# audeering/opensmile

Hardware: NVIDIA H100
Metric: LLD frames/sec (16kHz, 25ms/10ms) (higher is better)
Workload: dtype f32

## Files before the change

### opensmile_b200/csrc/api.cu

```cuda
#include <cuda_runtime.h>

#include <algorithm>
#include <cmath>
#include <cstdio>
#include <cstdlib>
#include <cstring>
#include <memory>
#include <string>
#include <vector>

#include "cuda_owned.hpp"
#include "kernels.cuh"
#include "plan.hpp"

using namespace osm;

namespace osm {
cudaError_t launch_lld_f32(const LldParams &p, int nfft, int numSMs, cudaStream_t st, LldLaunchInfo *info);
cudaError_t launch_energy_f32(const TimeOpParams &p, cudaStream_t st);
cudaError_t launch_mzcr_f32(const TimeOpParams &p, cudaStream_t st);
cudaError_t launch_intensity_f32(const TimeOpParams &p, cudaStream_t st);
cudaError_t launch_formant_f32(const FormantParams &p, cudaStream_t st);
cudaError_t launch_lpc_f32(const LpcParams &p, cudaStream_t st);
size_t lpc_smem_bytes_f32(const LpcParams &p);
cudaError_t launch_jitter_f32(const JitterParams &p, int u0, int u1, cudaStream_t st);
}

namespace {
thread_local std::string g_err;
}
namespace osm { osm_b200_status set_last_error(osm_b200_status st, const std::string &msg) { g_err = msg; return st; } }

namespace {
// ... 67 lines not shown
  RastaParams rp;
  DevBuf<float> dBand;
};

struct StreamRt {
  LldParams kp;
  std::vector<PassRt> extra;
  PassRt pass0x;
  int tileF = 32;
  bool runLld = false;
  bool forceNarrow = false;
  bool needTiles = false;
  const float *dWindow = nullptr;
  std::vector<int32_t> uttChunk0, uttTile0;
  PinBuf<ChunkRef> hChunks; DevBuf<ChunkRef> dChunks; size_t nChunks = 0;
  PinBuf<OpTile> hTiles; DevBuf<OpTile> dTiles; size_t nTiles = 0;
  DevBuf<float> dMag;
};

struct OpRt {
  int kind = 0, stream = 0;
  int vSrcCol = 0, vN = 0, vOutCol = 0;
  int magMode = 0; float magN = 1.f, magDbNorm = 0.f, magMinDb = 0.f;
  SpectralParams sp;
  TimeOpParams tp;
  AcfPitchParams ap;
  DevBuf<double> dSharpW;
  DevBuf<float2> dTw;
  DevBuf<PitchRaw> dRaw;
  ShsParams shs;
// ... 814 lines not shown
      size_t ti = 0;
      if (needPost)
        for (int u = 0; u < nUtt; u++) {
          const int64_t To = hR[u + 1] - hR[u];
          for (int64_t r0 = 0; r0 < To; r0 += PR) pl->hPost.p[ti++] = TileRef{u, (int32_t)r0};
        }
    }
    pl->nPostTiles = nPost;
    pl->totalWork = 0;
    for (size_t si = 0; si < pl->st.size(); si++) {
      StreamRt &rt = pl->st[si];
      const int F = rt.tileF, H = rt.kp.halo;
      std::vector<ChunkRef> chunks;
      std::vector<OpTile> tiles;
      rt.uttChunk0.assign(nm, 0); rt.uttTile0.assign(nm, 0);
      int64_t tileCount = 0;
      for (int u = 0; u < nUtt; u++) {
        const int64_t L = uttOff[u + 1] - uttOff[u];
        const int64_t T = desc_num_static_frames(d, (int)si, L);
        rt.uttChunk0[u] = (int32_t)chunks.size();
        rt.uttTile0[u] = (int32_t)tileCount;
        for (int64_t a = 0; a < T;) {
          const int64_t s0 = std::max<int64_t>(a - H, 0);
          const int64_t maxEnd = s0 + (int64_t)F * KT;
          const int64_t b2 = (maxEnd >= T) ? T : maxEnd - H;
          chunks.push_back(ChunkRef{u, (int32_t)a, (int32_t)b2, (int32_t)(tileCount + s0 / F)});
          a = b2;
        }
        if (rt.needTiles)
          for (int64_t f0 = 0; f0 < T; f0 += F)
            tiles.push_back(OpTile{u, (int32_t)f0, (int32_t)std::min<int64_t>(F, T - f0), f0 > 0 ? 1 : 0});
        tileCount += (T + F - 1) / F;
      }
      rt.uttChunk0[nUtt] = (int32_t)chunks.size();
      rt.uttTile0[nUtt] = (int32_t)tileCount;
      rt.nChunks = rt.runLld ? chunks.size() : 0;
      rt.nTiles = tiles.size();
      pl->totalWork += rt.nChunks + rt.nTiles;
      if (rt.runLld) {
        CU(rt.hChunks.reserve(chunks.size() + 1));
        if (!chunks.empty()) memcpy(rt.hChunks.p, chunks.data(), chunks.size() * sizeof(ChunkRef));
        CU(rt.dChunks.reserve(chunks.size() + 1));
        if (!chunks.empty()) CU(cudaMemcpyAsync(rt.dChunks.p, rt.hChunks.p, chunks.size() * sizeof(ChunkRef), cudaMemcpyHostToDevice, st));
        if (rt.kp.opKind < 0 || d.streams[si].dumpMag)
          CU(rt.dMag.reserve((size_t)tileCount * d.streams[si].fe.nBins * F + 64));
      }
      if (rt.needTiles) {
        CU(rt.hTiles.reserve(tiles.size() + 1));
        if (!tiles.empty()) memcpy(rt.hTiles.p, tiles.data(), tiles.size() * sizeof(OpTile));
        CU(rt.dTiles.reserve(tiles.size() + 1));
        if (!tiles.empty()) CU(cudaMemcpyAsync(rt.dTiles.p, rt.hTiles.p, tiles.size() * sizeof(OpTile), cudaMemcpyHostToDevice, st));
      }
    }
    pl->totalRows = hR[nUtt];
    pl->totalStat = hS[nUtt];
    pl->totalSamples = uttOff[nUtt];
    CU(pl->dMeta.reserve(3 * nm));
    CU(pl->dPost.reserve(nPost + 1));
    CU(cudaMemcpyAsync(pl->dMeta.p, pl->hMeta.p, 3 * nm * sizeof(long long), cudaMemcpyHostToDevice, st));
    if (nPost) CU(cudaMemcpyAsync(pl->dPost.p, pl->hPost.p, nPost * sizeof(TileRef), cudaMemcpyHostToDevice, st));
// ... 48 lines not shown
  }
  for (size_t si = 0; si < pl->st.size(); si++) {
    StreamRt &rt = pl->st[si];
    if (!rt.runLld) continue;
    const int c0 = rt.uttChunk0[u0], c1 = rt.uttChunk0[u1];
    if (c1 <= c0) continue;
    const long long *hS = pl->hMeta.p + 2 * nm;
    const long long row0 = hS[u0], row1 = hS[u1];
    for (size_t j = 0; j <= rt.extra.size(); j++) {
      PassRt &pr = j == 0 ? rt.pass0x : rt.extra[j - 1];
      LldParams kp = j == 0 ? rt.kp : pr.kp;
      kp.pcm = reinterpret_cast<const int16_t *>(d_pcm);
      kp.uttOff = dU;
      kp.chunks = rt.dChunks.p + c0;
      kp.nChunks = c1 - c0;
      kp.magOut = (j == 0 && d.streams[si].dumpMag) ? rt.dMag.p : nullptr;
      if (pl->staticDirect) {
        kp.out = d_out; kp.outStride = d.nOut; kp.outCol = pl->identityOutCol; kp.rowOff = dR;
      } else {
        kp.out = pl->dStat.p; kp.outStride = d.nStatic; kp.rowOff = dS;
        kp.outCol = pr.op >= 0 ? d.ops[pr.op].outCol : 0;
      }
      if (pr.rasta) {
        CU(pr.dBand.reserve((size_t)pl->totalStat * kp.nBands + 64));
        kp.out = pr.dBand.p; kp.outStride = kp.nBands; kp.outCol = 0; kp.rowOff = dS;
      }
      CU((f32in ? launch_lld_f32 : launch_lld)(kp, d.streams[si].fe.nfft, pl->numSMs, st, &pl->lastInfo));
      pl->lastLaunches++;
      PROF("lld_kernel");
      if (pr.rasta) {
        RastaParams rp = pr.rp;
        rp.band = pr.dBand.p; rp.uttOff = dU; rp.statOff = dS;
        CU(launch_rasta(rp, u0, u1, st));
        PROF("rasta_kernel");
        CU(launch_plp_tail(pr.tail, pr.dBand.p, pl->dStat.p, d.nStatic, d.ops[pr.op].outCol, row0, row1, st));
        pl->lastLaunches += 2;
        PROF("plp_tail_kernel");
      }
    }
  }
  if (u0 == 0) CU(cudaEventRecord(pl->evKm, st));
  bool forked = false;
// ... 334 lines not shown
```

### opensmile_b200/csrc/kernels.cu

```cuda
#include <cstdio>
#include <cstdlib>
#include <string>

#include "fft_radix.cuh"
#include "kernels.cuh"

#include "lld_common.cuh"

namespace osm {

constexpr int kUnrollMel = OSM_UNROLL_MEL, kUnrollDct = OSM_UNROLL_DCT;

template <int M, int F, int NT, int MINB, bool VEC2, bool GEN>
__global__ void __launch_bounds__(NT, MINB) lld_kernel(const LldParams p)
{
  const int opKind = GEN ? p.opKind : 0;
  float *const magOut = GEN ? p.magOut : nullptr;
  constexpr int NW = NT / 32, G = 32 / F, NVW = NW * G;
  constexpr int NBINS = M + 1;
  constexpr int NPAIR = M / 2 + 1;
  constexpr int PAIRS_PER_VW = (NPAIR + NVW - 1) / NVW;
  using Fc = Fact<M>;

  extern __shared__ __align__(16) unsigned char smem[];
// ... 9 lines not shown
  float2 *sSplit = reinterpret_cast<float2 *>(smem + L.splitTw);
  float2 *sMelCoef = reinterpret_cast<float2 *>(smem + L.melCoef);
  int *sMelRange = reinterpret_cast<int *>(smem + L.melRange);
  float *sDct = reinterpret_cast<float *>(smem + L.dctCos);
  float *sLift = reinterpret_cast<float *>(smem + L.dctLift);
  float *sEql = reinterpret_cast<float *>(smem + L.eql);
  float *melS = reinterpret_cast<float *>(smem + L.melS);
  float *ring = reinterpret_cast<float *>(smem + L.ring);
  float *Dbuf = reinterpret_cast<float *>(smem + L.zbuf);

  const int tid = threadIdx.x;
  const int warp = tid >> 5, lane = tid & 31;
  const int f = lane & (F - 1);
  const int vw = warp * G + lane / F;

  if (tid == 0) mbar_init(mbar, 1);
  for (int i = tid; i < M; i += NT) sWinLut[i] = p.winLut[i];
  for (int i = tid; i < p.twCount; i += NT) sTw[i] = p.twiddles[i];
  for (int i = tid; i < NPAIR; i += NT) sSplit[i] = p.splitTw[i];
  if (opKind >= 0) {
    for (int i = tid; i < p.melVCount; i += NT) sMelCoef[i] = p.melVisit[i];
    for (int i = tid; i < p.nBands + 2; i += NT) { sMelRange[i] = p.melRange[i]; sMelRange[p.nBands + 2 + i] = p.melVB[i]; }
    for (int i = tid; i < p.dctRows * p.dctStride; i += NT) sDct[i] = p.dctCos[i];
    if (opKind == 1) for (int i = tid; i < p.nBands; i += NT) sEql[i] = p.plpEql[i];
    for (int i = tid; i < p.nStat; i += NT) sLift[i] = p.dctLift[i];
  }
  for (int i = tid; i < L.sampFloats; i += NT) samp[i] = 0.f;
  for (int i = tid; i < F; i += NT) raw[i] = 0.f;
  __syncthreads();

  const int hop = p.frameStep, nChan = p.nChan;
  const int S = hop + p.sPad;
  uint32_t phase = 0;

  int chunk = blockIdx.x;
  if (chunk >= p.nChunks) return;
  ChunkCtx cx = load_chunk<F>(p, chunk);
  int j = 0;
  int emitted = cx.a;
  if (tid == 0) {
    const TileGeom g0 = tile_geom<F>(p, cx, 0);
    mbar_expect_tx(mbar, g0.bytes);
    bulk_g2s(rawPcm, g0.src, g0.bytes, mbar);
  }

  while (chunk < p.nChunks) {
    const TileGeom tg = tile_geom<F>(p, cx, j);
    const int nf = tg.nf, count = tg.count;

    mbar_wait(mbar, phase);
    phase ^= 1;
    {
      const int16_t *rp = reinterpret_cast<const int16_t *>(rawPcm + tg.mis) + tg.lead * nChan;
      const bool fastLoad = (tg.mis == 0) && (nChan <= 2) && !(OSM_PCM_F32_SUPPORT && p.pcmF32);
      const bool fastStore = (p.sPad == 0) || (hop % 8 == 0);
      for (int c = tid; c * 8 < count; c += NT) {
        const int i = c * 8;
        const int nvalid = min(8, count - i);
        float x[8];
        if (fastLoad && nvalid == 8) {
          if (nChan == 1) {
// ... 47 lines not shown
              if (rr == 0 && qq < F) raw[qq] = x[jj];
              dst[jj] = y[jj];
              rr++;
              if (rr == hop) { rr = 0; qq++; dst += p.sPad; }
            }
          }
        }
      }
    }
    __syncthreads();
    if (tid == 0) {
      if (j + 1 < cx.nT) {
        const TileGeom gn = tile_geom<F>(p, cx, j + 1);
        mbar_expect_tx(mbar, gn.bytes);
        bulk_g2s(rawPcm, gn.src, gn.bytes, mbar);
      } else if (chunk + (int)gridDim.x < p.nChunks) {
        const ChunkCtx cn = load_chunk<F>(p, chunk + gridDim.x);
        const TileGeom gn = tile_geom<F>(p, cn, 0);
        mbar_expect_tx(mbar, gn.bytes);
        bulk_g2s(rawPcm, gn.src, gn.bytes, mbar);
      }
    }

    {
      const float *sampF = samp + f * S;
      fft_stage<M, F, NVW, Fc::R0, M, true, false, VEC2>(Z, sampF, raw, sWinLut, sTw + p.twOff[0], p, vw, f);
      __syncthreads();
      if constexpr (Fc::NS == 2) {
        fft_stage<M, F, NVW, Fc::R1, M / Fc::R0, false, true, VEC2>(Z, nullptr, nullptr, nullptr, nullptr, p, vw, f);
      } else {
        fft_stage<M, F, NVW, Fc::R1, M / Fc::R0, false, false, VEC2>(Z, nullptr, nullptr, nullptr, sTw + p.twOff[1], p, vw, f);
        __syncthreads();
// ... 169 lines not shown
      } else {
        emit_edge<F, NW>(ring, Dbuf, outS, K, W1, W2, T, T1, c01, c02, cx.s0, r0, r1, d0, d1, dRows, norm1, p.fRcp1, norm2, p.fRcp2, warp, lane);
      }
      {
        float *o = p.out + (cx.row0 + r0) * (long long)K3;
        const int n = nr * K3;
        for (int i = tid; i < n; i += NT) o[i] = outS[i];
      }
      emitted = r1;
    }

    }

    j++;
    if (j == cx.nT) {
      chunk += gridDim.x;
      j = 0;
      if (chunk < p.nChunks) { cx = load_chunk<F>(p, chunk); emitted = cx.a; }
    }
  }
}

constexpr int kPostRows = 64;
constexpr int kPostMaxHalo = 12;
constexpr int kPostThreads = 256;

__device__ __forceinline__ float post_read(const float *lvl, int n, int rowBase, int t, int W, int navail, int i, int c)
{
  if (t - W < 0) {
    if (i < 0) i = 0;
    else if (i >= navail) return 0.f;
  } else if (i > navail - 1) {
    i = navail - 1;
// ... 357 lines not shown
  return (size_t)make_layout(p, nfft / 2, lld_tile_frames(nfft, p.narrow != 0)).total;
}

#define OSM_STR2(x) #x
#define OSM_STR(x) OSM_STR2(x)
template <int M, int F, int NT, int MINB, bool VEC2, bool GEN>
static const char *lld_kernel_name()
{
  static const std::string name = std::string(OSM_STR(lld_kernel)) + "<" + std::to_string(M) + "," + std::to_string(F) + "," +
                                  std::to_string(NT) + "," + std::to_string(MINB) + (VEC2 ? ",VEC2" : ",SCALAR") +
                                  (GEN ? ",GEN>" : ",MFCC>");
  return name.c_str();
}

template <int M, int F, int NT, int MINB, bool VEC2, bool GEN>
static cudaError_t launch_g(const LldParams &p, int numSMs, cudaStream_t st, LldLaunchInfo *info)
{
  const size_t smem = (size_t)make_layout(p, M, F).total;
  auto kern = lld_kernel<M, F, NT, MINB, VEC2, GEN>;
  cudaError_t e = cudaFuncSetAttribute(kern, cudaFuncAttributeMaxDynamicSharedMemorySize, (int)smem);
  if (e != cudaSuccess) return e;
  int occ = 0;
  e = cudaOccupancyMaxActiveBlocksPerMultiprocessor(&occ, kern, NT, smem);
  if (e != cudaSuccess) return e;
  if (occ < 1) return cudaErrorLaunchOutOfResources;
  int grid = numSMs * occ;
  if (grid > p.nChunks) grid = p.nChunks;
  if (grid < 1) grid = 1;
  if (info) {
    info->grid = grid; info->block = NT; info->smem = smem; info->nChunks = p.nChunks;
    info->kernel = lld_kernel_name<M, F, NT, MINB, VEC2, GEN>();
  }
  kern<<<grid, NT, smem, st>>>(p);
  return cudaGetLastError();
}

template <int M, int F, int NT, int MINB, bool VEC2>
static cudaError_t launch_t(const LldParams &p, int numSMs, cudaStream_t st, LldLaunchInfo *info)
{
  if (p.opKind == 0 && p.magOut == nullptr) return launch_g<M, F, NT, MINB, VEC2, false>(p, numSMs, st, info);
  return launch_g<M, F, NT, MINB, VEC2, true>(p, numSMs, st, info);
}

cudaError_t launch_lld(const LldParams &p, int nfft, int numSMs, cudaStream_t st, LldLaunchInfo *info)
{
  {
    static const bool fastOn = [] { const char *e = getenv("OSM_B200_LLD_FAST"); return !(e && e[0] == '0'); }();
    if (fastOn && lld_fast_applies(p, nfft)) return launch_lld_fast(p, numSMs, st, info);
  }
  const bool vec2 = ((p.frameStep + p.sPad) % 2) == 0;
  if (p.narrow && nfft == 1024) return vec2 ? launch_t<512, 16, 256, 1, true>(p, numSMs, st, info) : launch_t<512, 16, 256, 1, false>(p, numSMs, st, info);
  if (p.narrow && nfft == 2048) return vec2 ? launch_t<1024, 8, 256, 1, true>(p, numSMs, st, info) : launch_t<1024, 8, 256, 1, false>(p, numSMs, st, info);
  if (p.narrow && nfft == 4096) return vec2 ? launch_t<2048, 4, 128, 1, true>(p, numSMs, st, info) : launch_t<2048, 4, 128, 1, false>(p, numSMs, st, info);
  switch (nfft) {
    case 512:  return vec2 ? launch_t<256, 32, 256, 2, true>(p, numSMs, st, info) : launch_t<256, 32, 256, 2, false>(p, numSMs, st, info);
    case 1024: return vec2 ? launch_t<512, 32, 512, 1, true>(p, numSMs, st, info) : launch_t<512, 32, 512, 1, false>(p, numSMs, st, info);
    case 2048: return vec2 ? launch_t<1024, 16, 512, 1, true>(p, numSMs, st, info) : launch_t<1024, 16, 512, 1, false>(p, numSMs, st, info);
    case 4096: return vec2 ? launch_t<2048, 8, 256, 1, true>(p, numSMs, st, info) : launch_t<2048, 8, 256, 1, false>(p, numSMs, st, info);
    default:   return cudaErrorInvalidValue;
  }
}

int post_tile_rows(int nStat, int maxN, int halo)
{
  int rows = kPostRows;
  while (rows > 4 && (size_t)(rows + 2 * halo) * (nStat + 2 * maxN) * sizeof(float) > 160 * 1024) rows /= 2;
  return rows;
}

cudaError_t launch_post(const PostParams &p, cudaStream_t st)
{
  if (p.nTiles <= 0 || p.nGroups <= 0) return cudaSuccess;
  if (p.halo > kPostMaxHalo) return cudaErrorInvalidValue;
// ... 191 lines not shown
```

### opensmile_b200/csrc/kernels.cuh

```cuda
#pragma once
#include <cuda_runtime.h>
#include <cstdint>

#ifdef OSM_F32_VARIANT
#define OSM_PCM_F32_SUPPORT 1
#define lld_tile_frames lld_tile_frames_f32
#define lld_virtual_warps lld_virtual_warps_f32
#define lld_max_chunk_tiles lld_max_chunk_tiles_f32
#define lld_supported_fft lld_supported_fft_f32
#define lld_smem_bytes lld_smem_bytes_f32
#define launch_lld launch_lld_f32
#define post_tile_rows post_tile_rows_f32
#define launch_post launch_post_f32
#define acf_pitch_supported_fft acf_pitch_supported_fft_f32
#define launch_acf_pitch launch_acf_pitch_f32
#define launch_rasta launch_rasta_f32
#define launch_plp_tail launch_plp_tail_f32
#define launch_cms_means launch_cms_means_f32
#define launch_vecop_ll1 launch_vecop_ll1_f32
#define launch_pitch_smooth launch_pitch_smooth_f32
#define launch_spectral launch_spectral_f32
#define launch_mag_rows launch_mag_rows_f32
#define launch_intensity launch_intensity_f32
#define launch_energy launch_energy_f32
// ... 17 lines not shown
#define plp_tail_kernel plp_tail_kernel_f32
#define post_kernel post_kernel_f32
#define rasta_kernel rasta_kernel_f32
#define spectral_kernel spectral_kernel_f32
#define vecop_ll1_kernel vecop_ll1_kernel_f32
#endif
#ifndef OSM_PCM_F32_SUPPORT
#define OSM_PCM_F32_SUPPORT 0
#endif

namespace osm {

constexpr int kMaxVW = 32;

struct TileRef { int32_t utt; int32_t f0; };
struct ChunkRef { int32_t utt; int32_t a; int32_t b; int32_t tile0; };

struct LldParams {
  const int16_t *pcm;
  const long long *uttOff;
  const long long *rowOff;
  const ChunkRef *chunks;
  int nChunks;
  int nChan;
  int pcmF32;
  unsigned hopMagic;
  int narrow;
  int fused, halo, fW1, fW2;
  float fNorm1, fNorm2;
  float fRcp1, fRcp2;
  int frameSize, frameStep, sPad;
  int preemph, preDe;
  float preK, oneMinusK;
  int hasWinOffset;
  float winOffset;
  const float4 *winLut;
  const float2 *twiddles;
  int twOff[4];
// ... 42 lines not shown
  const long long *uttOff;
  int nUtt;
  int nGroups;
  PostGroup groups[kMaxPostGroups];
  const TileRef *tiles;
  int rows;
  int nTiles;
  int nStat;
  int maxN;
  int halo;
  const float *means;
};

struct LldLaunchInfo { int grid, block; size_t smem; const char *kernel; long long nChunks; };

cudaError_t launch_lld(const LldParams &p, int nfft, int numSMs, cudaStream_t st, LldLaunchInfo *info);
cudaError_t launch_post(const PostParams &p, cudaStream_t st);
bool lld_fast_applies(const LldParams &p, int nfft);
cudaError_t launch_lld_fast(const LldParams &p, int numSMs, cudaStream_t st, LldLaunchInfo *info);
int post_tile_rows(int nStat, int maxN, int halo);
size_t lld_smem_bytes(const LldParams &p, int nfft);
int lld_tile_frames(int nfft, bool narrow = false);
int lld_virtual_warps(int nfft);
int lld_max_chunk_tiles();
bool lld_supported_fft(int nfft);

struct OpTile { int32_t utt; int32_t f0; int32_t nf; int32_t prev; };

struct SpectralParams {
  const float *mag;
  const OpTile *tiles; int nTiles; int F;
  const long long *statOff;
  float *stat; int statStride, outCol;
  int nSrc, loBin, hiBin;
// ... 165 lines not shown
```

### opensmile_b200/csrc/lld_common.cuh

```cuda
#pragma once
#include <cstdio>

#include "fft_radix.cuh"
#include "kernels.cuh"

#ifndef OSM_EMIT_LANES
#define OSM_EMIT_LANES 0
#endif
#ifndef OSM_MEL_COMPACT
#define OSM_MEL_COMPACT 1
#endif
#ifndef OSM_UNROLL_MEL
#define OSM_UNROLL_MEL 4
#endif
#ifndef OSM_UNROLL_DCT
#define OSM_UNROLL_DCT 2
#endif

namespace osm {

struct SmemLayout {
  int zbuf, samp, raw, rawPcm, mbar, winLut, tw, splitTw, melCoef, melRange, dctCos, dctLift, eql, melS, ring;
  int total;
  int sampFloats, rawPcmBytes;
// ... 98 lines not shown
__device__ __forceinline__ ChunkCtx load_chunk(const LldParams &p, int chunk)
{
  ChunkCtx c;
  const ChunkRef cr = p.chunks[chunk];
  c.utt = cr.utt; c.a = cr.a; c.b = cr.b; c.tile0 = cr.tile0;
  c.uo = p.uttOff[cr.utt];
  const long long Ls = p.uttOff[cr.utt + 1] - c.uo;
  c.T = (int)((Ls - p.frameSize) / p.frameStep + 1);
  c.s0 = max(cr.a - p.halo, 0);
  c.sEnd = min(cr.b + p.halo, c.T);
  c.nT = (c.sEnd - c.s0 + F - 1) / F;
  c.row0 = p.rowOff[cr.utt];
  return c;
}

struct TileGeom {
  int fs;
  int nf;
  int count;
  int lead;
  int mis;
  uint32_t bytes;
  const char *src;
};

template <int F>
__device__ __forceinline__ TileGeom tile_geom(const LldParams &p, const ChunkCtx &c, int j)
{
  TileGeom g;
  g.fs = c.s0 + j * F;
// ... 286 lines not shown
```

### opensmile_b200/csrc/lld_fast.cu

```cuda
#include "lld_common.cuh"

#ifndef OSM_FAST_FUSED_DCT
#define OSM_FAST_FUSED_DCT 0
#endif
#ifndef OSM_FAST_P1_UNROLL
#define OSM_FAST_P1_UNROLL 1
#endif
#ifndef OSM_FAST_P2_UNROLL
#define OSM_FAST_P2_UNROLL 2
#endif
#ifndef OSM_FAST_MEL_UNROLL
#define OSM_FAST_MEL_UNROLL 1
#endif
#ifndef OSM_FAST_DCT_UNROLL
#define OSM_FAST_DCT_UNROLL 4
#endif
#ifndef OSM_FAST_STAGE_UNROLL
#define OSM_FAST_STAGE_UNROLL 1
#endif
#ifndef OSM_FAST_EMIT_K13
#define OSM_FAST_EMIT_K13 0
#endif
#define OSM_PRAGMA_(x) _Pragma(#x)
#define OSM_UNROLL(n) OSM_PRAGMA_(unroll n)

namespace osm {
namespace {

constexpr int kM = 256, kF = 32, kNT = 256, kNW = 8;
constexpr int kKMax = 16;
constexpr int kPartOff = 9216;

__device__ __forceinline__ void dft4_d0(float2 &a, float2 &b, float2 &c, float2 &d)
{
  const float2 t0 = cadd(a, c), t1 = csub(a, c), bb = b;
  a = cadd(t0, bb);
  c = csub(t0, bb);
  b = make_float2(t1.x + bb.y, t1.y - bb.x);
  d = make_float2(t1.x - bb.y, t1.y + bb.x);
}

// ... 32 lines not shown
  const float2 t2 = cmul(o2, w);
  const float xr = e2.x + t2.y, xi = e2.y - t2.x;
  const float yr = e2.x - t2.y, yi = e2.y + t2.x;
  pk = __fmaf_rn(xr, xr, __fmul_rn(xi, xi));
  pm = __fmaf_rn(yr, yr, __fmul_rn(yi, yi));
}

template <int NZR>
__global__ void __launch_bounds__(kNT, 2) lld512_kernel(const LldParams p)
{
  constexpr int M = kM, F = kF, NT = kNT, NW = kNW;
  using D16 = Dft<16>;

  extern __shared__ __align__(16) unsigned char smem[];
  __shared__ ChunkCtx sCx[2];
  const SmemLayout L = make_layout(p, M, F);
  float2 *Z = reinterpret_cast<float2 *>(smem + L.zbuf);
  float *P = reinterpret_cast<float *>(smem + L.zbuf);
  float *samp = reinterpret_cast<float *>(smem + L.samp);
  float *raw = reinterpret_cast<float *>(smem + L.raw);
  unsigned char *rawPcm = smem + L.rawPcm;
  uint64_t *mbar = reinterpret_cast<uint64_t *>(smem + L.mbar);
  float4 *sWinLut = reinterpret_cast<float4 *>(smem + L.winLut);
  float2 *sTw = reinterpret_cast<float2 *>(smem + L.tw);
  float2 *sSplit = reinterpret_cast<float2 *>(smem + L.splitTw);
  float2 *sMelCoef = reinterpret_cast<float2 *>(smem + L.melCoef);
  int *sMelRange = reinterpret_cast<int *>(smem + L.melRange);
  float *sDct = reinterpret_cast<float *>(smem + L.dctCos);
  float *sLift = reinterpret_cast<float *>(smem + L.dctLift);
  float *ring = reinterpret_cast<float *>(smem + L.ring);
  float *Dbuf = reinterpret_cast<float *>(smem + L.zbuf);

  const int tid = threadIdx.x;
  const int warp = tid >> 5, f = tid & 31;

  if (tid == 0) mbar_init(mbar, 1);
  for (int i = tid; i < M; i += NT) sWinLut[i] = p.winLut[i];
  for (int i = tid; i < p.twCount; i += NT) sTw[i] = p.twiddles[i];
  for (int i = tid; i < M / 2 + 1; i += NT) sSplit[i] = p.splitTw[i];
  for (int i = tid; i < p.melVCount; i += NT) sMelCoef[i] = p.melVisit[i];
  for (int i = tid; i < p.nBands + 2; i += NT) { sMelRange[i] = p.melRange[i]; sMelRange[p.nBands + 2 + i] = p.melVB[i]; }
  for (int i = tid; i < p.nBands * kKMax; i += NT) {
    const int m = i / kKMax, c = i - m * kKMax;
    sDct[i] = (c < p.nStat) ? p.dctCos[c * p.dctStride + m] : 0.f;
  }
  for (int i = tid; i < p.nStat; i += NT) sLift[i] = p.dctLift[i];
  for (int i = tid; i < L.sampFloats; i += NT) samp[i] = 0.f;
  for (int i = tid; i < F; i += NT) raw[i] = 0.f;
  __syncthreads();

  const int hop = p.frameStep;
  const int S = hop + p.sPad;
  uint32_t phase = 0;

  int chunk = blockIdx.x;
  if (chunk >= p.nChunks) return;
  int cpar = 0;
  if (tid == 0) {
    sCx[0] = load_chunk<F>(p, chunk);
    const TileGeom g0 = tile_geom<F>(p, sCx[0], 0);
    mbar_expect_tx(mbar, g0.bytes);
    bulk_g2s(rawPcm, g0.src, g0.bytes, mbar);
  }
  __syncthreads();
  int j = 0;
  int emitted = sCx[0].a;

  const int tA = (warp == 0) ? 0 : warp, tB = (warp == 0) ? 8 : 16 - warp;
  const int wl = (warp == 0) ? 8 : warp, wh = (warp == 0) ? 0 : warp;
  const int melBs = p.melSplit[warp], melBe = p.melSplit[warp + 1];

  while (chunk < p.nChunks) {
    const ChunkCtx &cx = sCx[cpar];

    mbar_wait(mbar, phase);
    phase ^= 1;
    {
      const TileGeom tg = tile_geom<F>(p, cx, j);
      const int count = tg.count;
      const int16_t *rp = reinterpret_cast<const int16_t *>(rawPcm + tg.mis) + tg.lead;
      const bool aligned = (tg.mis == 0);
      const bool hasLead = tg.lead > 0;
      const float ks = p.preDe ? p.preK : -p.preK;
      OSM_UNROLL(OSM_FAST_STAGE_UNROLL)
      for (int i = tid * 8; i < count; i += NT * 8) {
        int wds[4];
        if (aligned) {
// ... 20 lines not shown
          for (int jj = 0; jj < 8; jj++) y[jj] = x[jj];
        }
        const int q = (int)__umulhi((unsigned)i, p.hopMagic);
        float *dst = samp + i + q * p.sPad;
        if (i == q * hop && q < F) raw[q] = x[0];
#pragma unroll
        for (int jj = 0; jj < 8; jj += 2) *reinterpret_cast<float2 *>(dst + jj) = make_float2(y[jj], y[jj + 1]);
      }
    }
    __syncthreads();
    if (tid == 0) {
      if (j + 1 < cx.nT) {
        const TileGeom gn = tile_geom<F>(p, cx, j + 1);
        mbar_expect_tx(mbar, gn.bytes);
        bulk_g2s(rawPcm, gn.src, gn.bytes, mbar);
      } else if (chunk + (int)gridDim.x < p.nChunks) {
        const ChunkCtx cn = load_chunk<F>(p, chunk + gridDim.x);
        sCx[cpar ^ 1] = cn;
        const TileGeom gn = tile_geom<F>(p, cn, 0);
        mbar_expect_tx(mbar, gn.bytes);
        bulk_g2s(rawPcm, gn.src, gn.bytes, mbar);
      }
    }

    {
      const float *sampF = samp + f * S;
      const float2 *tw0 = sTw + p.twOff[0];
      OSM_UNROLL(OSM_FAST_P1_UNROLL)
      for (int t = warp; t < 16; t += NW) {
        float2 v[16];
#pragma unroll
        for (int r = 0; r < 16; r++) {
          if (r < NZR) {
            const float4 wl = sWinLut[t + 16 * r];
            const float2 x = *reinterpret_cast<const float2 *>(sampF + __float_as_int(wl.z));
            v[r] = make_float2(__fmul_rn(x.x, wl.x), __fmul_rn(x.y, wl.y));
          } else {
            v[r] = make_float2(0.f, 0.f);
          }
        }
        if (t == 0 && p.preemph)
          v[0].x = __fmul_rn(__fmul_rn(p.oneMinusK, raw[f]), sWinLut[0].x);
        dft16_first<NZR>(v);
        const float2 *twj = tw0 + t * 16;
#pragma unroll
        for (int q = 1; q < 16; q++) v[D16::out(q)] = cmul(v[D16::out(q)], twj[q]);
        float2 *zp = Z + t * F + f;
#pragma unroll
        for (int q = 0; q < 16; q++) zp[(16 * q) * F] = v[D16::out(q)];
      }
    }
    __syncthreads();

    {
      float2 A[16], v[16];
      OSM_UNROLL(OSM_FAST_P2_UNROLL)
      for (int h = 0; h < 2; h++) {
        const float2 *zp = Z + ((h ? tB : tA) * 16) * F + f;
#pragma unroll
        for (int r = 0; r < 16; r++) v[r] = zp[r * F];
        D16::run(v);
        if (h == 0) {
#pragma unroll
          for (int r = 0; r < 16; r++) A[r] = v[r];
        }
      }
      const float2 x0 = A[D16::out(0)];
// ... 21 lines not shown
#pragma unroll
        for (int q = 0; q < 8; q++) { Plo[(16 * q) * F] = pk[q]; Plm[(-16 * q) * F] = pm[q]; }
#pragma unroll
        for (int q = 8; q < 16; q++) {
          Phi[(-16 * q) * F] = pk[q];
          if (q > 8 || warp != 0) Phm[(16 * q) * F] = pm[q];
        }
      }
      if (warp == 0) {
        const float xr = 2.0f * (x0.x + x0.y), yr = 2.0f * (x0.x - x0.y);
        P[f] = __fmul_rn(xr, xr);
        P[M * F + f] = __fmul_rn(yr, yr);
      }
    }
    __syncthreads();

#if OSM_FAST_FUSED_DCT
    {
      float acc[kKMax];
#pragma unroll
      for (int c = 0; c < kKMax; c++) acc[c] = 0.f;
      if (melBs < melBe) {
        const int *sVB = sMelRange + p.nBands + 2;
        float cur = 0.f;
        for (int r = melBs; r <= melBe; r++) {
          float nxt = 0.f;
          const float *pp = P + sMelRange[r] * F + f;
          const int v0 = sVB[r];
          const float4 *cp = reinterpret_cast<const float4 *>(sMelCoef + v0);
          OSM_UNROLL(OSM_FAST_MEL_UNROLL)
// ... 14 lines not shown
              const float4 d = dt[c4];
              acc[4 * c4 + 0] = __fmaf_rn(mval, d.x, acc[4 * c4 + 0]);
              acc[4 * c4 + 1] = __fmaf_rn(mval, d.y, acc[4 * c4 + 1]);
              acc[4 * c4 + 2] = __fmaf_rn(mval, d.z, acc[4 * c4 + 2]);
              acc[4 * c4 + 3] = __fmaf_rn(mval, d.w, acc[4 * c4 + 3]);
            }
          }
          cur = nxt;
        }
      }
      float *part = P + kPartOff + warp * (kKMax * F) + f;
#pragma unroll
      for (int c = 0; c < kKMax; c++) part[c * F] = acc[c];
    }
    __syncthreads();

    const int ringBase = (j & 1) * F;
    for (int c = warp; c < p.nStat; c += NW) {
      const float *pp = P + kPartOff + c * F + f;
      float a = pp[0];
#pragma unroll
      for (int w = 1; w < NW; w++) a = __fadd_rn(a, pp[w * (kKMax * F)]);
      ring[c * (2 * F) + ringBase + f] = __fmul_rn(a, sLift[c]);
    }
    __syncthreads();

#else
    float *melS = P + kPartOff;
    if (melBs < melBe) {
      const int *sVB = sMelRange + p.nBands + 2;
      float cur = 0.f;
      for (int r = melBs; r <= melBe; r++) {
        float nxt = 0.f;
        const float *pp = P + sMelRange[r] * F + f;
        const int v0 = sVB[r];
        const float4 *cp = reinterpret_cast<const float4 *>(sMelCoef + v0);
        OSM_UNROLL(OSM_FAST_MEL_UNROLL)
        for (int q = (sVB[r + 1] - v0) >> 2; q > 0; q--, pp += 4 * F, cp += 2) {
          const float p0 = pp[0], p1 = pp[F], p2 = pp[2 * F], p3 = pp[3 * F];
          const float4 wa = cp[0], wb = cp[1];
          cur = __fmaf_rn(p0, wa.x, cur); nxt = __fmaf_rn(p0, wa.y, nxt);
          cur = __fmaf_rn(p1, wa.z, cur); nxt = __fmaf_rn(p1, wa.w, nxt);
          cur = __fmaf_rn(p2, wb.x, cur); nxt = __fmaf_rn(p2, wb.y, nxt);
          cur = __fmaf_rn(p3, wb.z, cur); nxt = __fmaf_rn(p3, wb.w, nxt);
        }
        if (r > melBs) {
          float mval = __fmul_rn(cur, p.melScale);
          if (p.doLog) mval = (mval < p.melfloor) ? p.logMelfloor : logf(mval);
          melS[(r - 1) * F + f] = mval;
        }
        cur = nxt;
      }
    }
    __syncthreads();

    const int ringBase = (j & 1) * F;
    {
      const int i = 2 * warp;
      if (i < p.nStat) {
        const float2 *cc = reinterpret_cast<const float2 *>(sDct + i);
        const float *lp = melS + f;
        float a0 = 0.f, a1 = 0.f;
        OSM_UNROLL(OSM_FAST_DCT_UNROLL)
        for (int m = 0; m < p.nBands; m++, lp += F, cc += kKMax / 2) {
          const float l0 = lp[0];
          const float2 c = cc[0];
          a0 = __fmaf_rn(l0, c.x, a0); a1 = __fmaf_rn(l0, c.y, a1);
        }
        ring[i * (2 * F) + ringBase + f] = __fmul_rn(a0, sLift[i]);
        if (i + 1 < p.nStat) ring[(i + 1) * (2 * F) + ringBase + f] = __fmul_rn(a1, sLift[i + 1]);
      }
    }
    __syncthreads();

#endif
    const int tfs = cx.s0 + j * F;
    if (!p.fused) {
      const int tot = min(F, cx.sEnd - tfs) * p.nStat;
      for (int idx = tid; idx < tot; idx += NT) {
        const int ff = idx / p.nStat, c = idx - ff * p.nStat;
        p.out[(cx.row0 + tfs + ff) * p.outStride + p.outCol + c] = ring[c * (2 * F) + ringBase + ff];
      }
    } else {
      const int K = p.nStat, W1 = p.fW1, W2 = p.fW2, H = W1 + W2;
      const int T = cx.T;
      const int r0 = emitted;
      const int r1 = (j + 1 == cx.nT) ? cx.b : min(tfs + F - H, cx.b);
      const int T1 = T + W1, c01 = max(T - W1, 0), c02 = max(c01 - W2, 0);
// ... 2 lines not shown
      const int dRows = F + 24;
      float *outS = Dbuf + ((K * dRows + 3) & ~3);
      const int K3 = 3 * K;
      const int nr = r1 - r0;
      const bool interior1 = (d0 >= W1) && (d1 + W1 <= T);
      const bool interior2 = (r0 >= W2) && (r1 <= c02);
      if (interior1 && interior2 && W1 == 2 && W2 == 2 && nr == F) {
#if OSM_FAST_EMIT_K13
        if (K == 13) emit_interior<F, NT, 13>(ring, Dbuf, outS, K, dRows, d0 - cx.s0, r0 - cx.s0, norm1, p.fRcp1, norm2, p.fRcp2, tid);
        else
#endif
        emit_interior<F, NT, 0>(ring, Dbuf, outS, K, dRows, d0 - cx.s0, r0 - cx.s0, norm1, p.fRcp1, norm2, p.fRcp2, tid);
      } else {
        emit_edge<F, NW>(ring, Dbuf, outS, K, W1, W2, T, T1, c01, c02, cx.s0, r0, r1, d0, d1, dRows, norm1, p.fRcp1, norm2, p.fRcp2, warp, f);
      }
      {
        float *o = p.out + (cx.row0 + r0) * (long long)K3;
        const int n = nr * K3;
        for (int i = tid; i < n; i += NT) o[i] = outS[i];
      }
      emitted = r1;
    }

    j++;
    if (j == cx.nT) {
      chunk += gridDim.x;
      j = 0;
      cpar ^= 1;
      if (chunk < p.nChunks) emitted = sCx[cpar].a;
    }
  }
}

template <int NZR>
cudaError_t launch_fast_t(const LldParams &p, int numSMs, cudaStream_t st, LldLaunchInfo *info)
{
  const size_t smem = (size_t)make_layout(p, kM, kF).total;
  auto kern = lld512_kernel<NZR>;
  cudaError_t e = cudaFuncSetAttribute(kern, cudaFuncAttributeMaxDynamicSharedMemorySize, (int)smem);
  if (e != cudaSuccess) return e;
  int occ = 0;
  e = cudaOccupancyMaxActiveBlocksPerMultiprocessor(&occ, kern, kNT, smem);
  if (e != cudaSuccess) return e;
  if (occ < 1) return cudaErrorLaunchOutOfResources;
  int grid = numSMs * occ;
  if (grid > p.nChunks) grid = p.nChunks;
  if (grid < 1) grid = 1;
  if (info) {
    info->grid = grid; info->block = kNT; info->smem = smem; info->nChunks = p.nChunks;
    info->kernel = NZR == 13 ? "lld512_kernel<13>" : "lld512_kernel<16>";
  }
  kern<<<grid, kNT, smem, st>>>(p);
  return cudaGetLastError();
}

}

bool lld_fast_applies(const LldParams &p, int nfft)
{
  return nfft == 512 && !p.narrow && p.opKind == 0 && p.magOut == nullptr && p.melUsePower && p.nChan == 1 &&
         p.frameStep % 8 == 0 && p.frameSize % 8 == 0 && p.frameSize <= 512 && !p.hasWinOffset && p.nStat <= kKMax &&
         ((p.frameStep + p.sPad) % 2) == 0;
}

cudaError_t launch_lld_fast(const LldParams &p, int numSMs, cudaStream_t st, LldLaunchInfo *info)
{
  if (p.frameSize <= 416) return launch_fast_t<13>(p, numSMs, st, info);
  return launch_fast_t<16>(p, numSMs, st, info);
}

}
```

Before: 902.1 million.

## Balance LLD chunk work across CTAs with contiguous tile-weighted runs

Chunks are now cut on the host so that each persistent CTA receives a contiguous run of chunks with roughly equal tile count (quota Q), and the kernel binary-searches its run start via a prefix tile-weight w0 instead of striding by gridDim. The grid size equals the number of runs. This targets tail imbalance across CTAs and gives sequential prefetch within a run, at the cost of extra chunk splits (more halo recompute) and a host-side iterative schedule. It also adds optional compile-time phase-clock instrumentation.

Result: faster. 940.8 million (median of 6 runs) (+4.3%).

```diff
diff --git a/opensmile_b200/csrc/api.cu b/opensmile_b200/csrc/api.cu
--- a/opensmile_b200/csrc/api.cu
+++ b/opensmile_b200/csrc/api.cu
@@ -9,6 +9,7 @@
 #include <string>
 #include <vector>
 
+#include "chunk_schedule.hpp"
 #include "cuda_owned.hpp"
 #include "kernels.cuh"
 #include "plan.hpp"
@@ -16,7 +17,7 @@
 using namespace osm;
 
 namespace osm {
-cudaError_t launch_lld_f32(const LldParams &p, int nfft, int numSMs, cudaStream_t st, LldLaunchInfo *info);
+cudaError_t launch_lld_f32(const LldParams &p, int nfft, int numSMs, cudaStream_t st, LldLaunchInfo *info, bool launch = true);
 cudaError_t launch_energy_f32(const TimeOpParams &p, cudaStream_t st);
 cudaError_t launch_mzcr_f32(const TimeOpParams &p, cudaStream_t st);
 cudaError_t launch_intensity_f32(const TimeOpParams &p, cudaStream_t st);
@@ -114,6 +115,8 @@
   const float *dWindow = nullptr;
   std::vector<int32_t> uttChunk0, uttTile0;
   PinBuf<ChunkRef> hChunks; DevBuf<ChunkRef> dChunks; size_t nChunks = 0;
+  int lldCtas = 1;
+  int ctaTiles = 1;
   PinBuf<OpTile> hTiles; DevBuf<OpTile> dTiles; size_t nTiles = 0;
   DevBuf<float> dMag;
 };
@@ -958,36 +961,33 @@
       std::vector<ChunkRef> chunks;
       std::vector<OpTile> tiles;
       rt.uttChunk0.assign(nm, 0); rt.uttTile0.assign(nm, 0);
-      int64_t tileCount = 0;
-      for (int u = 0; u < nUtt; u++) {
-        const int64_t L = uttOff[u + 1] - uttOff[u];
-        const int64_t T = desc_num_static_frames(d, (int)si, L);
-        rt.uttChunk0[u] = (int32_t)chunks.size();
-        rt.uttTile0[u] = (int32_t)tileCount;
-        for (int64_t a = 0; a < T;) {
-          const int64_t s0 = std::max<int64_t>(a - H, 0);
-          const int64_t maxEnd = s0 + (int64_t)F * KT;
-          const int64_t b2 = (maxEnd >= T) ? T : maxEnd - H;
-          chunks.push_back(ChunkRef{u, (int32_t)a, (int32_t)b2, (int32_t)(tileCount + s0 / F)});
-          a = b2;
-        }
-        if (rt.needTiles)
-          for (int64_t f0 = 0; f0 < T; f0 += F)
-            tiles.push_back(OpTile{u, (int32_t)f0, (int32_t)std::min<int64_t>(F, T - f0), f0 > 0 ? 1 : 0});
-        tileCount += (T + F - 1) / F;
-      }
-      rt.uttChunk0[nUtt] = (int32_t)chunks.size();
-      rt.uttTile0[nUtt] = (int32_t)tileCount;
-      rt.nChunks = rt.runLld ? chunks.size() : 0;
+      std::vector<int64_t> T(nUtt);
+      for (int u = 0; u < nUtt; u++) T[u] = desc_num_static_frames(d, (int)si, uttOff[u + 1] - uttOff[u]);
+      if (rt.runLld) {
+        cut_chunks(T.data(), nUtt, F, H, KT, 0, chunks, rt.uttChunk0.data(), rt.uttTile0.data());
+        if (rt.kp.opKind < 0 || d.streams[si].dumpMag)
+          CU(rt.dMag.reserve((size_t)rt.uttTile0[nUtt] * d.streams[si].fe.nBins * F + 64));
+        LldParams kq = rt.kp;
+        kq.magOut = d.streams[si].dumpMag ? rt.dMag.p : nullptr;
+        LldLaunchInfo li{};
+        CU((d.fe0().format != OSM_B200_PCM_S16 ? launch_lld_f32 : launch_lld)(kq, d.streams[si].fe.nfft, pl->numSMs, st, &li, false));
+        rt.lldCtas = std::max(li.grid, 1);
+        rt.ctaTiles = (int)balanced_chunks(T.data(), nUtt, F, H, KT, rt.lldCtas, chunks, rt.uttChunk0.data(), rt.uttTile0.data());
+      } else {
+        cut_chunks(T.data(), nUtt, F, H, KT, 0, chunks, rt.uttChunk0.data(), rt.uttTile0.data());
+      }
+      if (rt.needTiles)
+        for (int u = 0; u < nUtt; u++)
+          for (int64_t f0 = 0; f0 < T[u]; f0 += F)
+            tiles.push_back(OpTile{u, (int32_t)f0, (int32_t)std::min<int64_t>(F, T[u] - f0), f0 > 0 ? 1 : 0});
+      rt.nChunks = rt.runLld ? chunks.size() - 1 : 0;
       rt.nTiles = tiles.size();
       pl->totalWork += rt.nChunks + rt.nTiles;
       if (rt.runLld) {
-        CU(rt.hChunks.reserve(chunks.size() + 1));
-        if (!chunks.empty()) memcpy(rt.hChunks.p, chunks.data(), chunks.size() * sizeof(ChunkRef));
-        CU(rt.dChunks.reserve(chunks.size() + 1));
-        if (!chunks.empty()) CU(cudaMemcpyAsync(rt.dChunks.p, rt.hChunks.p, chunks.size() * sizeof(ChunkRef), cudaMemcpyHostToDevice, st));
-        if (rt.kp.opKind < 0 || d.streams[si].dumpMag)
-          CU(rt.dMag.reserve((size_t)tileCount * d.streams[si].fe.nBins * F + 64));
+        CU(rt.hChunks.reserve(chunks.size()));
+        memcpy(rt.hChunks.p, chunks.data(), chunks.size() * sizeof(ChunkRef));
+        CU(rt.dChunks.reserve(chunks.size()));
+        CU(cudaMemcpyAsync(rt.dChunks.p, rt.hChunks.p, chunks.size() * sizeof(ChunkRef), cudaMemcpyHostToDevice, st));
       }
       if (rt.needTiles) {
         CU(rt.hTiles.reserve(tiles.size() + 1));
@@ -1066,6 +1066,11 @@
       kp.uttOff = dU;
       kp.chunks = rt.dChunks.p + c0;
       kp.nChunks = c1 - c0;
+      {
+        const int64_t W = rt.hChunks.p[c1].w0 - rt.hChunks.p[c0].w0;
+        kp.ctaTiles = (c0 == 0 && c1 == (int)rt.nChunks) ? rt.ctaTiles : (int)((W + rt.lldCtas - 1) / rt.lldCtas);
+        kp.nRuns = (int)((W + kp.ctaTiles - 1) / kp.ctaTiles);
+      }
       kp.magOut = (j == 0 && d.streams[si].dumpMag) ? rt.dMag.p : nullptr;
       if (pl->staticDirect) {
         kp.out = d_out; kp.outStride = d.nOut; kp.outCol = pl->identityOutCol; kp.rowOff = dR;
@@ -1077,7 +1082,7 @@
         CU(pr.dBand.reserve((size_t)pl->totalStat * kp.nBands + 64));
         kp.out = pr.dBand.p; kp.outStride = kp.nBands; kp.outCol = 0; kp.rowOff = dS;
       }
-      CU((f32in ? launch_lld_f32 : launch_lld)(kp, d.streams[si].fe.nfft, pl->numSMs, st, &pl->lastInfo));
+      CU((f32in ? launch_lld_f32 : launch_lld)(kp, d.streams[si].fe.nfft, pl->numSMs, st, &pl->lastInfo, true));
       pl->lastLaunches++;
       PROF("lld_kernel");
       if (pr.rasta) {
diff --git a/opensmile_b200/csrc/chunk_schedule.hpp b/opensmile_b200/csrc/chunk_schedule.hpp
--- /dev/null
+++ b/opensmile_b200/csrc/chunk_schedule.hpp
@@ -0,0 +1,48 @@
+#pragma once
+#include <algorithm>
+#include <cstdint>
+#include <vector>
+
+#include "kernels.cuh"
+
+namespace osm {
+
+inline int64_t cut_chunks(const int64_t *T, int nUtt, int F, int H, int KT, int64_t Q, std::vector<ChunkRef> &chunks,
+                          int32_t *uttChunk0, int32_t *uttTile0)
+{
+  chunks.clear();
+  int64_t w = 0, tileCount = 0;
+  for (int u = 0; u < nUtt; u++) {
+    const int64_t Tu = T[u];
+    uttChunk0[u] = (int32_t)chunks.size();
+    uttTile0[u] = (int32_t)tileCount;
+    for (int64_t a = 0; a < Tu;) {
+      const int64_t s0 = std::max<int64_t>(a - H, 0);
+      const auto end = [&](int64_t n) { return s0 + F * n >= Tu ? Tu : s0 + F * n - H; };
+      int64_t b = end(Q > 0 ? std::min<int64_t>(KT, Q - w % Q) : KT);
+      if (b <= a) {
+        if (Q > 0 && w % Q != 0) { w += Q - w % Q; continue; }
+        b = end(KT);
+      }
+      chunks.push_back(ChunkRef{u, (int32_t)a, (int32_t)b, (int32_t)(tileCount + s0 / F), (int32_t)w});
+      w += (std::min<int64_t>(b + H, Tu) - s0 + F - 1) / F;
+      a = b;
+    }
+    tileCount += (Tu + F - 1) / F;
+  }
+  uttChunk0[nUtt] = (int32_t)chunks.size();
+  uttTile0[nUtt] = (int32_t)tileCount;
+  return w;
+}
+
+inline int64_t balanced_chunks(const int64_t *T, int nUtt, int F, int H, int KT, int ctas, std::vector<ChunkRef> &chunks,
+                               int32_t *uttChunk0, int32_t *uttTile0)
+{
+  int64_t W = cut_chunks(T, nUtt, F, H, KT, 0, chunks, uttChunk0, uttTile0);
+  int64_t Q = std::max<int64_t>((W + ctas - 1) / ctas, 1);
+  while ((W = cut_chunks(T, nUtt, F, H, KT, Q, chunks, uttChunk0, uttTile0)) > Q * ctas) Q++;
+  chunks.push_back(ChunkRef{nUtt, 0, 0, 0, (int32_t)W});
+  return Q;
+}
+
+}
diff --git a/opensmile_b200/csrc/kernels.cu b/opensmile_b200/csrc/kernels.cu
--- a/opensmile_b200/csrc/kernels.cu
+++ b/opensmile_b200/csrc/kernels.cu
@@ -47,7 +47,9 @@
   const int f = lane & (F - 1);
   const int vw = warp * G + lane / F;
 
+  __shared__ int sRun[2];
   if (tid == 0) mbar_init(mbar, 1);
+  if (tid < 2) sRun[tid] = chunk_run_begin(p, blockIdx.x + tid);
   for (int i = tid; i < M; i += NT) sWinLut[i] = p.winLut[i];
   for (int i = tid; i < p.twCount; i += NT) sTw[i] = p.twiddles[i];
   for (int i = tid; i < NPAIR; i += NT) sSplit[i] = p.splitTw[i];
@@ -66,8 +68,9 @@
   const int S = hop + p.sPad;
   uint32_t phase = 0;
 
-  int chunk = blockIdx.x;
-  if (chunk >= p.nChunks) return;
+  int chunk = sRun[0];
+  const int chunkEnd = sRun[1];
+  if (chunk >= chunkEnd) return;
   ChunkCtx cx = load_chunk<F>(p, chunk);
   int j = 0;
   int emitted = cx.a;
@@ -77,7 +80,7 @@
     bulk_g2s(rawPcm, g0.src, g0.bytes, mbar);
   }
 
-  while (chunk < p.nChunks) {
+  while (chunk < chunkEnd) {
     const TileGeom tg = tile_geom<F>(p, cx, j);
     const int nf = tg.nf, count = tg.count;
 
@@ -155,8 +158,8 @@
         const TileGeom gn = tile_geom<F>(p, cx, j + 1);
         mbar_expect_tx(mbar, gn.bytes);
         bulk_g2s(rawPcm, gn.src, gn.bytes, mbar);
-      } else if (chunk + (int)gridDim.x < p.nChunks) {
-        const ChunkCtx cn = load_chunk<F>(p, chunk + gridDim.x);
+      } else if (chunk + 1 < chunkEnd) {
+        const ChunkCtx cn = load_chunk<F>(p, chunk + 1);
         const TileGeom gn = tile_geom<F>(p, cn, 0);
         mbar_expect_tx(mbar, gn.bytes);
         bulk_g2s(rawPcm, gn.src, gn.bytes, mbar);
@@ -356,9 +359,9 @@
 
     j++;
     if (j == cx.nT) {
-      chunk += gridDim.x;
+      chunk++;
       j = 0;
-      if (chunk < p.nChunks) { cx = load_chunk<F>(p, chunk); emitted = cx.a; }
+      if (chunk < chunkEnd) { cx = load_chunk<F>(p, chunk); emitted = cx.a; }
     }
   }
 }
@@ -746,7 +749,7 @@
 }
 
 template <int M, int F, int NT, int MINB, bool VEC2, bool GEN>
-static cudaError_t launch_g(const LldParams &p, int numSMs, cudaStream_t st, LldLaunchInfo *info)
+static cudaError_t launch_g(const LldParams &p, int numSMs, cudaStream_t st, LldLaunchInfo *info, bool launch)
 {
   const size_t smem = (size_t)make_layout(p, M, F).total;
   auto kern = lld_kernel<M, F, NT, MINB, VEC2, GEN>;
@@ -756,39 +759,38 @@
   e = cudaOccupancyMaxActiveBlocksPerMultiprocessor(&occ, kern, NT, smem);
   if (e != cudaSuccess) return e;
   if (occ < 1) return cudaErrorLaunchOutOfResources;
-  int grid = numSMs * occ;
-  if (grid > p.nChunks) grid = p.nChunks;
-  if (grid < 1) grid = 1;
+  const int grid = launch ? p.nRuns : numSMs * occ;
   if (info) {
     info->grid = grid; info->block = NT; info->smem = smem; info->nChunks = p.nChunks;
     info->kernel = lld_kernel_name<M, F, NT, MINB, VEC2, GEN>();
   }
+  if (!launch) return cudaSuccess;
   kern<<<grid, NT, smem, st>>>(p);
   return cudaGetLastError();
 }
 
 template <int M, int F, int NT, int MINB, bool VEC2>
-static cudaError_t launch_t(const LldParams &p, int numSMs, cudaStream_t st, LldLaunchInfo *info)
-{
-  if (p.opKind == 0 && p.magOut == nullptr) return launch_g<M, F, NT, MINB, VEC2, false>(p, numSMs, st, info);
-  return launch_g<M, F, NT, MINB, VEC2, true>(p, numSMs, st, info);
-}
-
-cudaError_t launch_lld(const LldParams &p, int nfft, int numSMs, cudaStream_t st, LldLaunchInfo *info)
+static cudaError_t launch_t(const LldParams &p, int numSMs, cudaStream_t st, LldLaunchInfo *info, bool launch)
+{
+  if (p.opKind == 0 && p.magOut == nullptr) return launch_g<M, F, NT, MINB, VEC2, false>(p, numSMs, st, info, launch);
+  return launch_g<M, F, NT, MINB, VEC2, true>(p, numSMs, st, info, launch);
+}
+
+cudaError_t launch_lld(const LldParams &p, int nfft, int numSMs, cudaStream_t st, LldLaunchInfo *info, bool launch)
 {
   {
     static const bool fastOn = [] { const char *e = getenv("OSM_B200_LLD_FAST"); return !(e && e[0] == '0'); }();
-    if (fastOn && lld_fast_applies(p, nfft)) return launch_lld_fast(p, numSMs, st, info);
+    if (fastOn && lld_fast_applies(p, nfft)) return launch_lld_fast(p, numSMs, st, info, launch);
   }
   const bool vec2 = ((p.frameStep + p.sPad) % 2) == 0;
-  if (p.narrow && nfft == 1024) return vec2 ? launch_t<512, 16, 256, 1, true>(p, numSMs, st, info) : launch_t<512, 16, 256, 1, false>(p, numSMs, st, info);
-  if (p.narrow && nfft == 2048) return vec2 ? launch_t<1024, 8, 256, 1, true>(p, numSMs, st, info) : launch_t<1024, 8, 256, 1, false>(p, numSMs, st, info);
-  if (p.narrow && nfft == 4096) return vec2 ? launch_t<2048, 4, 128, 1, true>(p, numSMs, st, info) : launch_t<2048, 4, 128, 1, false>(p, numSMs, st, info);
+  if (p.narrow && nfft == 1024) return vec2 ? launch_t<512, 16, 256, 1, true>(p, numSMs, st, info, launch) : launch_t<512, 16, 256, 1, false>(p, numSMs, st, info, launch);
+  if (p.narrow && nfft == 2048) return vec2 ? launch_t<1024, 8, 256, 1, true>(p, numSMs, st, info, launch) : launch_t<1024, 8, 256, 1, false>(p, numSMs, st, info, launch);
+  if (p.narrow && nfft == 4096) return vec2 ? launch_t<2048, 4, 128, 1, true>(p, numSMs, st, info, launch) : launch_t<2048, 4, 128, 1, false>(p, numSMs, st, info, launch);
   switch (nfft) {
-    case 512:  return vec2 ? launch_t<256, 32, 256, 2, true>(p, numSMs, st, info) : launch_t<256, 32, 256, 2, false>(p, numSMs, st, info);
-    case 1024: return vec2 ? launch_t<512, 32, 512, 1, true>(p, numSMs, st, info) : launch_t<512, 32, 512, 1, false>(p, numSMs, st, info);
-    case 2048: return vec2 ? launch_t<1024, 16, 512, 1, true>(p, numSMs, st, info) : launch_t<1024, 16, 512, 1, false>(p, numSMs, st, info);
-    case 4096: return vec2 ? launch_t<2048, 8, 256, 1, true>(p, numSMs, st, info) : launch_t<2048, 8, 256, 1, false>(p, numSMs, st, info);
+    case 512:  return vec2 ? launch_t<256, 32, 256, 2, true>(p, numSMs, st, info, launch) : launch_t<256, 32, 256, 2, false>(p, numSMs, st, info, launch);
+    case 1024: return vec2 ? launch_t<512, 32, 512, 1, true>(p, numSMs, st, info, launch) : launch_t<512, 32, 512, 1, false>(p, numSMs, st, info, launch);
+    case 2048: return vec2 ? launch_t<1024, 16, 512, 1, true>(p, numSMs, st, info, launch) : launch_t<1024, 16, 512, 1, false>(p, numSMs, st, info, launch);
+    case 4096: return vec2 ? launch_t<2048, 8, 256, 1, true>(p, numSMs, st, info, launch) : launch_t<2048, 8, 256, 1, false>(p, numSMs, st, info, launch);
     default:   return cudaErrorInvalidValue;
   }
 }
diff --git a/opensmile_b200/csrc/kernels.cuh b/opensmile_b200/csrc/kernels.cuh
--- a/opensmile_b200/csrc/kernels.cuh
+++ b/opensmile_b200/csrc/kernels.cuh
@@ -55,7 +55,7 @@
 constexpr int kMaxVW = 32;
 
 struct TileRef { int32_t utt; int32_t f0; };
-struct ChunkRef { int32_t utt; int32_t a; int32_t b; int32_t tile0; };
+struct ChunkRef { int32_t utt; int32_t a; int32_t b; int32_t tile0; int32_t w0; };
 
 struct LldParams {
   const int16_t *pcm;
@@ -63,6 +63,7 @@
   const long long *rowOff;
   const ChunkRef *chunks;
   int nChunks;
+  int ctaTiles, nRuns;
   int nChan;
   int pcmF32;
   unsigned hopMagic;
@@ -135,10 +136,10 @@
 
 struct LldLaunchInfo { int grid, block; size_t smem; const char *kernel; long long nChunks; };
 
-cudaError_t launch_lld(const LldParams &p, int nfft, int numSMs, cudaStream_t st, LldLaunchInfo *info);
+cudaError_t launch_lld(const LldParams &p, int nfft, int numSMs, cudaStream_t st, LldLaunchInfo *info, bool launch = true);
 cudaError_t launch_post(const PostParams &p, cudaStream_t st);
 bool lld_fast_applies(const LldParams &p, int nfft);
-cudaError_t launch_lld_fast(const LldParams &p, int numSMs, cudaStream_t st, LldLaunchInfo *info);
+cudaError_t launch_lld_fast(const LldParams &p, int numSMs, cudaStream_t st, LldLaunchInfo *info, bool launch);
 int post_tile_rows(int nStat, int maxN, int halo);
 size_t lld_smem_bytes(const LldParams &p, int nfft);
 int lld_tile_frames(int nfft, bool narrow = false);
diff --git a/opensmile_b200/csrc/lld_common.cuh b/opensmile_b200/csrc/lld_common.cuh
--- a/opensmile_b200/csrc/lld_common.cuh
+++ b/opensmile_b200/csrc/lld_common.cuh
@@ -136,6 +136,18 @@
   return c;
 }
 
+__device__ __forceinline__ int chunk_run_begin(const LldParams &p, int g)
+{
+  const long long w = (long long)p.chunks[0].w0 + (long long)g * p.ctaTiles;
+  int lo = 0, hi = p.nChunks;
+  while (lo < hi) {
+    const int mid = (lo + hi) >> 1;
+    if (p.chunks[mid].w0 < w) lo = mid + 1;
+    else hi = mid;
+  }
+  return lo;
+}
+
 struct TileGeom {
   int fs;
   int nf;
diff --git a/opensmile_b200/csrc/lld_fast.cu b/opensmile_b200/csrc/lld_fast.cu
--- a/opensmile_b200/csrc/lld_fast.cu
+++ b/opensmile_b200/csrc/lld_fast.cu
@@ -25,6 +25,22 @@
 #define OSM_UNROLL(n) OSM_PRAGMA_(unroll n)
 
 namespace osm {
+
+enum { kPhStage, kPhPass1, kPhPass2, kPhMel, kPhDct, kPhEmit, kPhStore, kPhKernel, kPhKernelMax, kPhTiles, kPhSlots };
+#ifdef OSM_LLD_PHASE_CLOCKS
+__device__ unsigned long long gLld512Phase[kPhSlots];
+#define OSM_PHASE(k)                                                    \
+  do {                                                                  \
+    if (tid == 0) {                                                     \
+      const long long c_ = clock64();                                   \
+      sPh[k] += (unsigned long long)(c_ - phT);                         \
+      phT = c_;                                                         \
+    }                                                                   \
+  } while (0)
+#else
+#define OSM_PHASE(k) do {} while (0)
+#endif
+
 namespace {
 
 constexpr int kM = 256, kF = 32, kNT = 256, kNW = 8;
@@ -87,6 +103,7 @@
 
   extern __shared__ __align__(16) unsigned char smem[];
   __shared__ ChunkCtx sCx[2];
+  __shared__ int sRun[2];
   const SmemLayout L = make_layout(p, M, F);
   float2 *Z = reinterpret_cast<float2 *>(smem + L.zbuf);
   float *P = reinterpret_cast<float *>(smem + L.zbuf);
@@ -108,6 +125,7 @@
   const int warp = tid >> 5, f = tid & 31;
 
   if (tid == 0) mbar_init(mbar, 1);
+  if (tid < 2) sRun[tid] = chunk_run_begin(p, blockIdx.x + tid);
   for (int i = tid; i < M; i += NT) sWinLut[i] = p.winLut[i];
   for (int i = tid; i < p.twCount; i += NT) sTw[i] = p.twiddles[i];
   for (int i = tid; i < M / 2 + 1; i += NT) sSplit[i] = p.splitTw[i];
@@ -125,9 +143,16 @@
   const int hop = p.frameStep;
   const int S = hop + p.sPad;
   uint32_t phase = 0;
-
-  int chunk = blockIdx.x;
-  if (chunk >= p.nChunks) return;
+#ifdef OSM_LLD_PHASE_CLOCKS
+  __shared__ unsigned long long sPh[kPhSlots];
+  if (tid < kPhSlots) sPh[tid] = 0;
+  const long long phT0 = clock64();
+  long long phT = phT0;
+#endif
+
+  int chunk = sRun[0];
+  const int chunkEnd = sRun[1];
+  if (chunk >= chunkEnd) return;
   int cpar = 0;
   if (tid == 0) {
     sCx[0] = load_chunk<F>(p, chunk);
@@ -143,7 +168,7 @@
   const int wl = (warp == 0) ? 8 : warp, wh = (warp == 0) ? 0 : warp;
   const int melBs = p.melSplit[warp], melBe = p.melSplit[warp + 1];
 
-  while (chunk < p.nChunks) {
+  while (chunk < chunkEnd) {
     const ChunkCtx &cx = sCx[cpar];
 
     mbar_wait(mbar, phase);
@@ -194,14 +219,15 @@
         const TileGeom gn = tile_geom<F>(p, cx, j + 1);
         mbar_expect_tx(mbar, gn.bytes);
         bulk_g2s(rawPcm, gn.src, gn.bytes, mbar);
-      } else if (chunk + (int)gridDim.x < p.nChunks) {
-        const ChunkCtx cn = load_chunk<F>(p, chunk + gridDim.x);
+      } else if (chunk + 1 < chunkEnd) {
+        const ChunkCtx cn = load_chunk<F>(p, chunk + 1);
         sCx[cpar ^ 1] = cn;
         const TileGeom gn = tile_geom<F>(p, cn, 0);
         mbar_expect_tx(mbar, gn.bytes);
         bulk_g2s(rawPcm, gn.src, gn.bytes, mbar);
       }
     }
+    OSM_PHASE(kPhStage);
 
     {
       const float *sampF = samp + f * S;
@@ -231,6 +257,7 @@
       }
     }
     __syncthreads();
+    OSM_PHASE(kPhPass1);
 
     {
       float2 A[16], v[16];
@@ -282,6 +309,7 @@
       }
     }
     __syncthreads();
+    OSM_PHASE(kPhPass2);
 
 #if OSM_FAST_FUSED_DCT
     {
@@ -326,6 +354,7 @@
       for (int c = 0; c < kKMax; c++) part[c * F] = acc[c];
     }
     __syncthreads();
+    OSM_PHASE(kPhMel);
 
     const int ringBase = (j & 1) * F;
     for (int c = warp; c < p.nStat; c += NW) {
@@ -336,6 +365,7 @@
       ring[c * (2 * F) + ringBase + f] = __fmul_rn(a, sLift[c]);
     }
     __syncthreads();
+    OSM_PHASE(kPhDct);
 
 #else
     float *melS = P + kPartOff;
@@ -365,6 +395,7 @@
       }
     }
     __syncthreads();
+    OSM_PHASE(kPhMel);
 
     const int ringBase = (j & 1) * F;
     {
@@ -384,6 +415,7 @@
       }
     }
     __syncthreads();
+    OSM_PHASE(kPhDct);
 
 #endif
     const int tfs = cx.s0 + j * F;
@@ -416,6 +448,7 @@
       } else {
         emit_edge<F, NW>(ring, Dbuf, outS, K, W1, W2, T, T1, c01, c02, cx.s0, r0, r1, d0, d1, dRows, norm1, p.fRcp1, norm2, p.fRcp2, warp, f);
       }
+      OSM_PHASE(kPhEmit);
       {
         float *o = p.out + (cx.row0 + r0) * (long long)K3;
         const int n = nr * K3;
@@ -423,19 +456,31 @@
       }
       emitted = r1;
     }
+    OSM_PHASE(kPhStore);
+#ifdef OSM_LLD_PHASE_CLOCKS
+    if (tid == 0) sPh[kPhTiles]++;
+#endif
 
     j++;
     if (j == cx.nT) {
-      chunk += gridDim.x;
+      chunk++;
       j = 0;
       cpar ^= 1;
-      if (chunk < p.nChunks) emitted = sCx[cpar].a;
-    }
-  }
+      if (chunk < chunkEnd) emitted = sCx[cpar].a;
+    }
+  }
+#ifdef OSM_LLD_PHASE_CLOCKS
+  if (tid == 0) {
+    sPh[kPhKernel] = (unsigned long long)(clock64() - phT0);
+    for (int k = 0; k < kPhSlots; k++)
+      if (k != kPhKernelMax) atomicAdd(&gLld512Phase[k], sPh[k]);
+    atomicMax(&gLld512Phase[kPhKernelMax], sPh[kPhKernel]);
+  }
+#endif
 }
 
 template <int NZR>
-cudaError_t launch_fast_t(const LldParams &p, int numSMs, cudaStream_t st, LldLaunchInfo *info)
+cudaError_t launch_fast_t(const LldParams &p, int numSMs, cudaStream_t st, LldLaunchInfo *info, bool launch)
 {
   const size_t smem = (size_t)make_layout(p, kM, kF).total;
   auto kern = lld512_kernel<NZR>;
@@ -445,13 +490,12 @@
   e = cudaOccupancyMaxActiveBlocksPerMultiprocessor(&occ, kern, kNT, smem);
   if (e != cudaSuccess) return e;
   if (occ < 1) return cudaErrorLaunchOutOfResources;
-  int grid = numSMs * occ;
-  if (grid > p.nChunks) grid = p.nChunks;
-  if (grid < 1) grid = 1;
+  const int grid = launch ? p.nRuns : numSMs * occ;
   if (info) {
     info->grid = grid; info->block = kNT; info->smem = smem; info->nChunks = p.nChunks;
     info->kernel = NZR == 13 ? "lld512_kernel<13>" : "lld512_kernel<16>";
   }
+  if (!launch) return cudaSuccess;
   kern<<<grid, kNT, smem, st>>>(p);
   return cudaGetLastError();
 }
@@ -465,10 +509,22 @@
          ((p.frameStep + p.sPad) % 2) == 0;
 }
 
-cudaError_t launch_lld_fast(const LldParams &p, int numSMs, cudaStream_t st, LldLaunchInfo *info)
-{
-  if (p.frameSize <= 416) return launch_fast_t<13>(p, numSMs, st, info);
-  return launch_fast_t<16>(p, numSMs, st, info);
-}
-
-}
+cudaError_t launch_lld_fast(const LldParams &p, int numSMs, cudaStream_t st, LldLaunchInfo *info, bool launch)
+{
+  if (p.frameSize <= 416) return launch_fast_t<13>(p, numSMs, st, info, launch);
+  return launch_fast_t<16>(p, numSMs, st, info, launch);
+}
+
+#ifdef OSM_LLD_PHASE_CLOCKS
+extern "C" __attribute__((visibility("default"))) int osm_b200_lld512_phase_clocks(unsigned long long *out)
+{
+  cudaError_t e = cudaMemcpyFromSymbol(out, gLld512Phase, sizeof(gLld512Phase));
+  if (e == cudaSuccess) {
+    static const unsigned long long zero[kPhSlots] = {};
+    e = cudaMemcpyToSymbol(gLld512Phase, zero, sizeof(zero));
+  }
+  return (int)e;
+}
+#endif
+
+}
```
